# mhozza/covest

Hardware: AMD Instinct MI355X
Metric: grid-point log-likelihood evals/s, repeat model, 10k-bin hist (higher is better)
Workload: dtype f64

## Files before the change

### covest_amd/csrc/band.h

```cpp
#pragma once
#include <math.h>

#ifndef COVEST_HD
#ifdef __HIPCC__
#define COVEST_HD __host__ __device__
#else
#define COVEST_HD
#endif
#endif

namespace covest {

constexpr double kBandLn = 56.0;
constexpr int kBandClasses = 8;
constexpr int kBandNewton = 2;

constexpr int kBandMinShared = 8;

struct Band {
    int step_lo, step_hi;
};

struct BandTile {
    double key_first, key_last, cls_first, cls_last;
};

COVEST_HD inline BandTile band_tile(const double *ln_rate, const double *ln_comb, double key_first, double key_last)
{
    BandTile t = {key_first, key_last, -INFINITY, -INFINITY};
    for (int s = 1; s < kBandClasses; ++s) {
        const double lc = ln_comb[s] - ln_comb[0], lr = ln_rate[s] - ln_rate[0];
        if (!(lc > -INFINITY))
            continue;
        const double a = lc + key_first * lr, b = lc + key_last * lr;
// ... 14 lines not shown
    const Band full = {0, n_steps};
    const double mu = -ln_1mq, L = rate0 + mu;
    if (!(rate0 > 0.0) || !(mu >= 0.0) || !(L < 1e300) || !(t.key_first >= 1.0) || !(t.key_last >= t.key_first) ||
        !(t.key_last < 16384.0) || o_ref_max < 3 || n_steps < 2)
        return full;
    const double mode = t.key_last * mth.rcp(L);
    double o_ref = floor(mode);
    o_ref = o_ref < 3.0 ? 3.0 : o_ref;
    o_ref = o_ref > (double)o_ref_max ? (double)o_ref_max : o_ref;
    const double inv_ref = mth.rcp(o_ref);
    double a = 2.0 * mode + 8.0;
    for (int it = 0; it < kBandNewton; ++it) {
        const double g = -(a - o_ref) * L + t.key_last * mth.ln(a * inv_ref) + kBandLn;
        const double dg = -L + t.key_last * mth.rcp(a);
        if (!(dg < 0.0))
            return full;
        a -= g * mth.rcp(dg);
        if (!(a > mode))
            return full;
    }
    const double o_edge = ceil(a) + 1.0;
    if (!(o_edge < 4.0 * (double)n_steps))
        return full;
    const int step_hi = ((int)o_edge + 2) >> 2;
    if (step_hi < 1 || step_hi >= n_steps)
        return full;
    const double o_drop = 1.0 + 4.0 * (double)step_hi, o_top = 4.0 * (double)n_steps;
    const double base = o_ref * rate0 - (o_drop - o_ref) * mu + kBandLn, ln_o = mth.ln(o_top * inv_ref);
    if (!(base + t.key_first * ln_o + t.cls_first <= 0.0) || !(base + t.key_last * ln_o + t.cls_last <= 0.0))
        return full;
    return Band{0, step_hi};
}

struct BandBytes {
    static constexpr int kSlots = 6, kNone = 255;
    unsigned w0 = ~0u, w1 = ~0u;
    COVEST_HD void set(int k, int step_hi)
    {
        const unsigned hi = (unsigned)(step_hi < kNone ? step_hi : kNone);
        if (k < 4)
            w0 = (w0 & ~(255u << (8 * k))) | (hi << (8 * k));
        else
            w1 = (w1 & ~(255u << (8 * (k - 4)))) | (hi << (8 * (k - 4)));
    }
    COVEST_HD int get(int k) const { return (int)(((k < 4 ? w0 >> (8 * k) : w1 >> (8 * (k - 4)))) & 255u); }
};

}
```

### covest_amd/csrc/factored_build.h

```cpp
#pragma once
#include "factored_diag.h"
#include "fastmath.h"
#include "streams.h"
#include "tiles.h"
#include "wave.h"

namespace covest {

struct BuildLane {
    int tid, ld;
    bool in_row;
    __device__ __forceinline__ double *column(double *dst) const { return dst + (in_row ? tid : 0); }
};

template <int N, bool SPO, bool STORE>
__device__ __forceinline__ double walk_tile(StreamSet<8> &st, bool in_row, double *row, int ld, const double *scal, double k0,
                                            double renorm)
{
    if (STORE && !in_row)
        return 0.0;
    double xx[8];
#pragma unroll
    for (int s = 0; s < 8; ++s) {
        double xs = st.x[s];
// ... 79 lines not shown
        }
        return 0.0;
    }
    double sum = 0.0;
    for (int b = 0; b < (STORE ? kTileBins : nb); ++b) {
        const double g = b < nb ? st.step() : 0.0;
        if ((SPO || !STORE) && b < nb)
            sum = fma(g, scal[b], sum);
        if (STORE && ln.in_row)
            colp[b * ln.ld] = g;
    }
    st.leave_tile(rc.renorm);
    return SPO ? sum * 0x1p476 : sum * (1.0 / kBasicScale);
}

__device__ __forceinline__ bool sum_item_matters(const TileView &tv, const StreamSet<8> &st, int first, int n)
{
    const int tl = first + n - 1;
    const TileRec ra = tv.rec[first], rb = tv.rec[tl];
    const double ka = ra.k0 - 1.0, kb = rb.k0 + (double)(rb.nb - 1);
    const double lga = ra.lgam_prev, lgb = rb.lgam_last;
    bool matters = false;
#pragma unroll
    for (int s = 0; s < 8; ++s) {
        if ((st.gone >> s) & 1u)
            continue;
        const double lx = st.an.lx(s), c = st.an.c(s);
        const double top = fmax(fma(ka, lx, c - lga), fma(kb, lx, c - lgb));
        matters = matters || !(top < StreamSet<8>::kSumWindowLn) || (st.x[s] >= ka - 1.0 && st.x[s] <= kb + 1.0);
    }
    return __any(matters);
}

template <bool TAIL, bool SPO>
__device__ __forceinline__ void build_item(const TileView &tv, const FactoredPlan &plan, StreamSet<8> &st, CompSum &so,
                                           bool &resync, int tid, int ld, bool in_row, Stamps &stamps, int it,
                                           bool seg_start, double *dst)
{
    const BuildLane ln = {tid, ld, in_row};
    const int first = TAIL ? __builtin_amdgcn_readfirstlane(tv.item_first[it]) : it;
    if (TAIL && tv.item_sum[it] != 0) {
        if (COVEST_SKIP_PHASE(plan, 1))
            return;
        const int n = __builtin_amdgcn_readfirstlane(tv.item_ntiles[it]);
        if (SPO) {
            if (!seg_start && !sum_item_matters(tv, st, first, n)) {
#pragma unroll
                for (int s = 0; s < 8; ++s)
                    st.v[s] = 0.0;
                resync = true;
                return;
            }
            for (int r = 0; r < n; ++r) {
                if (st.gone == 0xFFu && !(seg_start && r == 0))
                    break;
                so.add(build_tile<SPO, false>(tv, plan, st, ln, stamps, first + r, (seg_start && r == 0) || resync, nullptr));
                resync = false;
            }
            return;
        }
        double *colp = ln.column(dst);
        for (int r = 0; r < n; ++r) {
            const double gsum = build_tile<SPO, false>(tv, plan, st, ln, stamps, first + r, seg_start && r == 0, nullptr);
            if (ln.in_row)
                colp[r * ln.ld] = gsum;
        }
        for (int r = n; r < kTileBins; ++r)
            if (ln.in_row)
                colp[r * ln.ld] = 0.0;
    } else {
        const double tsum = build_tile<SPO, true>(tv, plan, st, ln, stamps, first, seg_start || (SPO && resync), dst);
        resync = false;
        if (SPO)
            so.add(tsum);
    }
}

}
```

### covest_amd/csrc/factored_diag.h

```cpp
#pragma once
#include <hip/hip_runtime.h>

#include "tiles.h"

namespace covest {

struct StampNames {
    enum Lap {
        kBuild,
        kContract,
        kLog,
        kWait,
        kShared,
        kZero,
        kEnter,
        kFirst,
    };
    enum Stage {
        kStart,
        kFetched,
        kStreams,
        kUnits,
        kWalked,
    };
};

#ifdef COVEST_DIAG
struct Stamps : StampNames {
    long long *out;
    int mode;
    long long t0 = 0, lap_sum[8] = {0, 0, 0, 0, 0, 0, 0, 0}, at[5] = {0, 0, 0, 0, 0};
    __device__ Stamps(const FactoredPlan &plan, int waves, int wave)
        : out(plan.diag ? plan.diag + ((int64_t)(blockIdx.x * gridDim.y + blockIdx.y) * waves + wave) * 8 : nullptr),
          mode(plan.skip_phases)
    {
        stage(kStart);
    }
    __device__ void stage(Stage s) { at[s] = (long long)clock64(); }
    __device__ void walk_begins()
    {
        if (out)
            t0 = (long long)clock64();
    }
    __device__ void lap(Lap which)
    {
        if (out) {
            const long long now = (long long)clock64();
            lap_sum[which] += now - t0;
            t0 = now;
        }
    }
    __device__ void count_zero_tile()
    {
        if (out)
            lap_sum[kZero] += 1;
    }
    template <int MU>
    __device__ void first_fragments(const double (&a0)[MU], const double (&wfirst)[MU])
    {
        if (out) {
            double sink = 0.0;
#pragma unroll
            for (int k = 0; k < MU; ++k)
                sink += a0[k] + wfirst[k];
            asm volatile("" ::"v"(sink));
            lap(kFirst);
        }
    }
    __device__ void barrier_passed(int p, int t_begin, int t_end, int lane)
    {
        if (out && (mode & 0x10000)) {
            const long long now = (long long)clock64();
            if (lane == 0) {
                const int grp = (mode & 0x20000) ? min(7, p - t_begin + 1)
                                                 : min(7, (p - t_begin + 1) * 8 / (t_end - t_begin + 1));
                out[grp] += now - t0;
            }
        }
        lap(kWait);
    }
    __device__ void dump_laps(int lane)
    {
        stage(kWalked);
        if (out && lane == 0 && !(mode & 0x50000))
            for (int i = 0; i < 8; ++i)
                out[i] = lap_sum[i];
    }
    __device__ void dump_stages(int lane)
    {
        if (out && (mode & 0x40000) && lane == 0) {
            const long long end = (long long)clock64();
            for (int s = 0; s < 4; ++s)
                out[s] = at[s + 1] - at[s];
            out[4] = end - at[kWalked];
            out[5] = end - at[kStart];
            out[6] = at[kStart];
            out[7] = end;
        }
    }
};
#else
struct Stamps : StampNames {
    __device__ Stamps(const FactoredPlan &, int, int) {}
    __device__ void stage(Stage) {}
    __device__ void walk_begins() {}
    __device__ void lap(Lap) {}
    __device__ void count_zero_tile() {}
    template <int MU>
    __device__ void first_fragments(const double (&)[MU], const double (&)[MU])
    {
    }
    __device__ void barrier_passed(int, int, int, int) {}
    __device__ void dump_laps(int) {}
    __device__ void dump_stages(int) {}
};
#endif

}
```

### covest_amd/csrc/host_common.cpp

```cpp
#include "factored_launch.h"
#include "host.h"

using namespace covest;

namespace {
thread_local std::string g_last_error;
}

namespace covest {

int set_error(int code, const std::string &msg)
{
    g_last_error = msg;
    return code;
}

int fail_hip(hipError_t e, const char *what)
{
    g_last_error = std::string(what) + ": " + hipGetErrorString(e);
    if (e == hipErrorOutOfMemory) {
        (void)hipGetLastError();
        return COVEST_E_NOMEM;
    }
    return (e == hipErrorNoDevice || e == hipErrorInvalidDevice || e == hipErrorInsufficientDriver)
// ... 285 lines not shown
LaunchRecordScope::LaunchRecordScope(LaunchRecord &r) : prev(tls_record)
{
    r.clear();
    tls_record = &r;
}
LaunchRecordScope::LaunchRecordScope(LaunchRecord &r, bool append) : prev(tls_record)
{
    if (!append)
        r.clear();
    tls_record = &r;
}
LaunchRecordScope::~LaunchRecordScope() { tls_record = prev; }

void record_launch(const char *name, int64_t launches)
{
    LaunchRecord *r = tls_record;
    if (!r || launches <= 0)
        return;
    for (int i = 0; i < r->n_entries; ++i)
        if (r->entries[i].name == name) {
            r->entries[i].launches += launches;
            return;
        }
    if (r->n_entries < (int)(sizeof r->entries / sizeof r->entries[0]))
        r->entries[r->n_entries++] = LaunchRecord::Entry{name, launches};
}

void record_factored_plan(const FactoredPlan &plan, int shared_tiles, bool long_part)
{
    LaunchRecord *r = tls_record;
    if (!r || r->n_plans >= (int)(sizeof r->plans / sizeof r->plans[0]))
        return;
    r->plans[r->n_plans++] = LaunchRecord::Plan{plan.n_threads, plan.n_buf,  plan.ld,        plan.n_qblocks,
                                                shared_tiles,   plan.n_pass, plan.list_mode, long_part};
}

int64_t launch_record_text(const LaunchRecord &r, char *buf, int64_t cap)
{
    std::string t;
    char line[256];
    for (int i = 0; i < r.n_entries; ++i) {
        std::snprintf(line, sizeof line, "launch %s %lld\n", r.entries[i].name, (long long)r.entries[i].launches);
        t += line;
    }
    for (int i = 0; i < r.n_plans; ++i) {
        const LaunchRecord::Plan &p = r.plans[i];
        std::snprintf(line, sizeof line,
                      "plan n_threads=%d n_buf=%d ld=%d n_qblocks=%d shared_tiles=%d long=%d n_pass=%d list_mode=%d\n",
                      p.n_threads, p.n_buf, p.ld, p.n_qblocks, p.shared_tiles, p.long_part ? 1 : 0, p.n_pass, p.list_mode);
        t += line;
    }
    if (buf && cap > 0) {
        const size_t n = std::min<size_t>(t.size(), (size_t)(cap - 1));
        std::memcpy(buf, t.data(), n);
        buf[n] = '\0';
    }
    return (int64_t)t.size();
}

}

extern "C" {

int64_t covest_compiled_variants(char *buf, int64_t cap)
{
    if (cap < 0 || (cap > 0 && !buf))
        return fail(COVEST_E_INVALID, "covest_compiled_variants: bad argument");
    std::string t;
    auto add = [&](const char *const *names, int n) {
        for (int i = 0; i < n; ++i) {
            t += names[i];
            t += '\n';
        }
    };
    for (const FactoredVariant &v : kFactoredVariantTable)
        add(&v.name, 1);
    add(kFactoredFinishNames, 2);
    add(kBasicVariantNames, kBasicVariants);
    add(kFixVariantNames, kFixVariants);
    add(kArgminVariantNames, kArgminVariants);
    add(kDerivVariantNames, kDerivVariants);
    if (buf && cap > 0) {
// ... 33 lines not shown
```

### covest_amd/csrc/kernels.h

```cpp
#pragma once
#include <hip/hip_runtime_api.h>

#include <cstddef>

#include "device_model.h"
#include "handback.h"
#include "kmer_plan.h"
#include "tiles.h"

namespace covest {

struct LaunchRecord {
    struct Entry {
        const char *name;
        int64_t launches;
    };
    struct Plan {
        int32_t n_threads, n_buf, ld, n_qblocks, shared_tiles, n_pass, list_mode;
        bool long_part;
    };
    Entry entries[16];
    int n_entries = 0;
    Plan plans[8];
    int n_plans = 0;
    void clear() { n_entries = n_plans = 0; }
};
void record_launch(const char *name, int64_t launches = 1);
void record_factored_plan(const FactoredPlan &plan, int shared_tiles, bool long_part);
struct LaunchRecordScope {
    explicit LaunchRecordScope(LaunchRecord &r);
    LaunchRecordScope(LaunchRecord &r, bool append);
    ~LaunchRecordScope();
    LaunchRecord *prev;
};
constexpr int kFactoredVariants = 10, kBasicVariants = 8, kFixVariants = 6, kArgminVariants = 3, kDerivVariants = 7;
extern const char *const kFactoredFinishNames[2];
extern const char *const kBasicVariantNames[kBasicVariants];
extern const char *const kFixVariantNames[kFixVariants];
extern const char *const kArgminVariantNames[kArgminVariants];
extern const char *const kDerivVariantNames[kDerivVariants];

hipError_t launch_ll_direct(const DevModel &m, const PointSource &src, int64_t n, double *out_ll,
                            double *out_p, hipStream_t stream, bool ref_overflow = false);

hipError_t launch_ll_basic(const DevModel &m, const TileView &tv, const PointSource &src, int64_t n,
                           double *out_ll, const SubList &sub_list, hipStream_t stream);

hipError_t launch_ll_factored(const DevModel &m, const TileView &tv, const FactoredPlan &plan,
                              double *out_ll, const SubList &sub_list, hipStream_t stream);

hipError_t launch_ll_finish_partials(const DevModel &m, const TileView &tv, const double *partial,
                                     const int32_t *first_item, const double *point_par, const int32_t *point_T,
// ... 207 lines not shown
```

### covest_amd/csrc/ll_factored.hip

```cpp
#include <hip/hip_runtime.h>

#include <algorithm>
#include <mutex>

#include "band.h"
#include "factored_build.h"
#include "factored_contract.h"
#include "factored_diag.h"
#include "factored_epilogue.h"
#include "factored_launch.h"
#include "factored_log.h"
#include "fastmath.h"
#include "handback.h"
#include "kernels.h"
#include "point_fetch.h"
#include "streams.h"
#include "wave.h"

namespace covest {

namespace {

template <int NT, int HU, bool TAIL, bool PLAIN, int LDC = 0>
__global__ __launch_bounds__(NT) void ll_factored_kernel(const DevModel m, const int32_t n_tiles, const int32_t n_items,
                                                         const double *__restrict__ tile_dbl,
                                                         const int32_t *__restrict__ tile_int,
                                                         const FactoredPlan plan,
                                                         double *__restrict__ out_ll, const SubList sub_list)
{
    const TileView tv = tile_view_from(n_tiles, n_items, tile_dbl, tile_int);
    constexpr int NW = NT / kWave;
    constexpr int MU = 2 * HU;
    static_assert(MU == 6, "contract loops are written for 6 slots");
    constexpr bool SPO = PLAIN && TAIL;
    constexpr bool NEED_SCAL = !PLAIN;
    constexpr int LOG_DEG = PLAIN ? 3 : 5;
    const int LD = LDC ? LDC : plan.ld;
    constexpr int NE = FactoredLds::entries_of(NT);
    const FactoredLds lay{NT, plan.n_buf, LD, SPO};
    extern __shared__ double Gs[];
    __shared__ __attribute__((aligned(16))) double log_tab[kLogTableDoubles];
    __shared__ unsigned sub_rec[NE * 2];
    __shared__ __attribute__((aligned(16))) double2 rowc[2][kTileBins];
    __shared__ __attribute__((aligned(16))) double rows[NEED_SCAL ? 2 : 1][NEED_SCAL ? kTileBins : 2];
    __shared__ __attribute__((aligned(16))) double rho_tab[PLAIN ? NW * MU * 4 : 4];
    __shared__ double lconst_s;
    __shared__ double band_ln[PLAIN ? kBandClasses : 1];
    static_assert(MU == kMaxUnits, "the LDS layout counts kMaxUnits slots a wave");
    static_assert(sizeof(log_tab) + sizeof(sub_rec) + sizeof(rowc) + sizeof(rows) + sizeof(rho_tab) + sizeof(lconst_s) +
                          sizeof(band_ln) + 7 * 15 <= kFactoredStaticLds, "the planners' LDS budget (tiles.h) must hold the kernel's static LDS");

    const int tid = threadIdx.x;
    const int lane = tid & (kWave - 1);
    const int wave = __builtin_amdgcn_readfirstlane(tid / kWave);
    Stamps stamps(plan, NW, wave);
    const double p_clamp = plan.p_clamp;
    const double zero_frac = kZeroSteps * (kGridStep / p_clamp);
    const int list_mode = PLAIN ? 0 : plan.list_mode;

    const int n_seg = list_mode ? plan.n_seg : 1;
    const int unit = list_mode ? (int)blockIdx.x / n_seg : (int)blockIdx.x;
    const int seg = list_mode ? (int)blockIdx.x - unit * n_seg : 0;
    const int seg_items = (n_items + n_seg - 1) / n_seg;
    const int t_begin = seg * seg_items, t_end = min(n_items, t_begin + seg_items);
    const int64_t ce = (PLAIN || list_mode == 0) ? plan.ce_end - 1 - unit : plan.ce_begin + unit;
    const bool list = list_mode == 1 || list_mode == 2;
    const int64_t ic = list ? ce : ce / plan.n_e;
    const int64_t ie = list ? ce : ce - ic * plan.n_e;
    double par[kMaxParams] = {plan.c_axis[ic], plan.e_axis[ie], 0, 0, 0};
    constexpr int kLogPerThread = (kLogTableDoubles + NT - 1) / NT;
    double log_v[kLogPerThread];
#pragma unroll
    for (int u = 0; u < kLogPerThread; ++u)
        log_v[u] = kLogTable[min(tid + u * NT, kLogTableDoubles - 1)];
    const double rho_v = PLAIN ? plan.unit_rho[(int64_t)blockIdx.y * NW * MU * 4 + min(tid, NW * MU * 4 - 1)] : 0.0;
    double lc_first = 0.0;
    if (wave == NW - 1 && t_begin + lane < t_end)
        lc_first = tv.item_lconst[t_begin + lane];
#pragma unroll
    for (int u = 0; u < kLogPerThread; ++u)
        if (tid + u * NT < kLogTableDoubles)
            log_tab[tid + u * NT] = log_v[u];
    if (PLAIN && tid < NW * MU * 4)
// ... 1 lines not shown
#pragma unroll
    for (int u = 0; u < (NE + NT - 1) / NT; ++u)
        if (tid + u * NT < NE) {
            sub_rec[2 * (tid + u * NT)] = 0xFFFFFFFFu;
            sub_rec[2 * (tid + u * NT) + 1] = 0;
        }
    clamp_point<2>(m, par);
    const bool finite = isfinite(par[0]) && isfinite(par[1]);
    const int n_pass = PLAIN ? 1 : plan.n_pass;
    if (tid < 8 * n_pass)
        Gs[lay.rates() + tid] = error_class_rate_mul(m, par[0], par[1], tid, m.n_err);
    if (wave == NW - 1) {
        double lc = 0.0 + lc_first;
        for (int t = t_begin + lane + kWave; t < t_end; t += kWave)
            lc += tv.item_lconst[t];
        lc = wave_sum(lc);
        if (lane == 0)
            lconst_s = PLAIN ? lc - kLogRawBias<kScaleBits> * tv.suf_h[0] : lc;
    }
    __syncthreads();
    stamps.stage(Stamps::kFetched);

    const int my_pass = n_pass == 1 ? 0 : tid / plan.pass_stride;
    const int o_local = n_pass == 1 ? tid : tid - my_pass * plan.pass_stride;
    const bool wave_builds = wave * kWave < plan.n_columns;
    const int o_base = PLAIN ? 0 : list_mode == 2 ? plan.item_obase[ce] : plan.o_base;
    const int o_mine = o_base + o_local + 1;
    double lam[8];
#pragma unroll
    for (int s = 0; s < 8; ++s)
        lam[s] = Gs[lay.rates() + 8 * my_pass + s];
    if (PLAIN && tid < kBandClasses)
        band_ln[tid] = fast_log(Gs[lay.rates() + tid], log_tab);
    double n_total = -1.0;
    if (n_pass > 1) {
        n_total = 0.0;
        for (int s = 0; s < 8 * n_pass; ++s)
            n_total += m.comb[s] * (1.0 - exp_neg_rn((double)o_mine * Gs[lay.rates() + s]));
    }
    __syncthreads();
    StreamSet<8> st;
    if (wave_builds) {
        st.template init<false>(m, lam, o_mine, finite && my_pass < n_pass && o_local < plan.max_o, log_tab,
                                log_tab, 8 * my_pass, n_total);
    } else {
        st.gone = 0u;
#pragma unroll
        for (int s = 0; s < 8; ++s) {
            st.v[s] = 0.0;
            st.x[s] = 0.0;
            st.an.set(s, 0.0, -INFINITY);
        }
    }
    stamps.stage(Stamps::kStreams);
    const bool lane_in_row = tid < LD - 2;
    if (tid < FactoredLds::kSlack)
        Gs[lay.slack() + tid] = 0.0;
    if (tid < lay.rows()) {
        Gs[lay.pad(tid)] = 0.0;
        Gs[lay.pad(tid) + 1] = 0.0;
    }

    const int col = lane & 15;
    const int kq = lane >> 4;
    int len[MU], cont[MU], uhalf[MU], qslot[MU], cut[MU], a_off0[MU], nsh[MU];
    double r4[MU], llacc[MU];
// ... 29 lines not shown
        u_T[k] = plan.q_T[slot];
        r4[k] = plan.q_r4[slot];
    }
#pragma unroll
    for (int k = 0; k < MU; ++k) {
        const bool on = qslot[k] >= 0;
        const int first_step = __builtin_amdgcn_readfirstlane(u_s0[k]);
        len[k] = __builtin_amdgcn_readfirstlane(u_len[k]);
        cont[k] = __builtin_amdgcn_readfirstlane(u_cont[k]);
        uhalf[k] = __builtin_amdgcn_readfirstlane(u_half[k]);
        nsh[k] = PLAIN ? __builtin_amdgcn_readfirstlane(u_nsh[k]) : 0;
        a_off0[k] = (16 * uhalf[k] + col) * LD + kq + 4 * first_step;
        const int t_lane = on ? u_T[k] : 0;
        const int o0 = __builtin_amdgcn_readfirstlane(u_o0[k]);
        cut[k] = ((t_lane - (o0 + kq) + 3) >> 2) - nsh[k];
        llacc[k] = 0.0;
        dead[k] = 0;
        spacc[(TAIL && !SPO) ? k : 0].hi = 0.0;
        spacc[(TAIL && !SPO) ? k : 0].lo = 0.0;
    }

    unsigned m_first = 0, m_cont = 0, m_sh = 0;
#pragma unroll
    for (int k = 0; k < MU; ++k) {
        m_first |= (qslot[k] >= 0 && !cont[k]) ? 1u << k : 0u;
        m_cont |= cont[k] ? 1u << k : 0u;
        m_sh |= nsh[k] > 0 ? 1u << k : 0u;
    }
    BandBytes bands;
    bool wave_bands = false;
#pragma unroll
    for (int k = 0; k < MU; ++k)
        wave_bands = wave_bands || (PLAIN && !wave_builds && nsh[k] >= kBandMinShared);
    if (PLAIN && wave_bands) {
        struct {
            const double *tab;
            __device__ double ln(double x) const { return fast_log(x, tab); }
            __device__ double rcp(double x) const
            {
                const double r = __builtin_amdgcn_rcp(x);
                return fma(fma(-x, r, 1.0), r, r);
            }
        } const mth = {log_tab};
        const int it = min(lane, t_end - 1);
        const double key_first = tv.rec[TAIL ? tv.item_first[it] : it].k0;
        const double key_last = (lane < kWave - 1 ? key_first : tv.rec[n_tiles - 1].k0) + (double)(kTileBins - 1);
        const BandTile bt = band_tile(band_ln, m.ln_comb, key_first, key_last);
#pragma unroll
        for (int k = 0; k < MU; ++k) {
            if (nsh[k] < kBandMinShared)
                continue;
            const Band b = band_of_unit(mth, lam[0], rho_tab[4 * (wave * MU + k) + 1], 4 + 4 * nsh[k], nsh[k] + len[k], bt);
            bands.set(k, b.step_hi);
        }
    }
    double wfirst[MU], wrun[MU];
    auto load_weights = [&]() {
#pragma unroll
        for (int k = 0; k < MU; ++k) {
            const double2 pw = reinterpret_cast<const double2 *>(plan.piece_w)[(int64_t)(slot_base + k) * kWave + lane];
            wfirst[k] = pw.x;
            wrun[k] = pw.y;
        }
    };
    load_weights();

    bool resync = false;
    auto build = [&](int it, bool seg_start, double *dst) __attribute__((always_inline)) {
        build_item<TAIL, SPO>(tv, plan, st, so, resync, tid, LD, lane_in_row, stamps, it, seg_start, dst);
    };
    stamps.walk_begins();
    stamps.stage(Stamps::kUnits);

    const bool dbuf = plan.n_buf == 2;
    double nxt_h = 0.0, nxt_c = 0.0, nxt_s = 0.0;
    auto fetch_rows = [&](int it) {
        if (tid < kTileBins && it < t_end) {
            const int64_t at = (int64_t)it * kTileBins + tid;
            nxt_h = tv.item_cnt[at];
            nxt_c = tv.item_iscal[at];
            if (NEED_SCAL)
                nxt_s = tv.item_scal[at];
        }
    };
    int last_item = t_end - 1;
    if (SPO)
        while (last_item > t_begin && tv.item_sum[last_item] != 0)
            --last_item;
    const bool last_first = PLAIN && t_end - t_begin >= 2 && last_item > t_begin;
    auto tile_at = [&](int p) -> int { return last_first ? (p == t_begin ? last_item : (p <= last_item ? p - 1 : p)) : p; };
    const int t_endx = t_end + (SPO ? 1 : 0);
    fetch_rows(tile_at(t_begin));
    for (int p = t_begin - (dbuf ? 1 : 0); p < t_endx; ++p) {
        const int pb = dbuf ? p + 1 : p;
        if (SPO && pb == t_end) {
            if (wave_builds && lane_in_row) {
                double *dst = Gs + lay.buf(pb) + tid;
                dst[0] = so.hi * 0x1p-540;
                dst[LD] = so.lo * 0x1p-540;
            }
        } else if (pb < t_end) {
            if (tid < kTileBins) {
                rowc[pb & 1][tid] = make_double2(nxt_h, p_clamp * nxt_c);
                if (NEED_SCAL)
                    rows[pb & 1][tid] = nxt_s;
            }
            fetch_rows(pb + 1 < t_end ? tile_at(pb + 1) : t_end);
            if (wave_builds) {
                if (last_first && pb == t_begin + 1)
                    st.gone = 0u;
                build(tile_at(pb), pb == t_begin || (last_first && (pb == t_begin + 1 || pb == last_item + 1)), Gs + lay.buf(pb));
            }
        }
        stamps.lap(Stamps::kBuild);
        if (!dbuf)
            __syncthreads();
        const bool sp_item = SPO && p == t_end;
        if (p >= t_begin && !(SPO && !sp_item && tv.item_sum[tile_at(p)] != 0)) {
            const int t = tile_at(p);
            const double *cur = Gs + lay.buf(p);
            d4 acc[MU];
            const d4 zero4 = (d4){0.0, 0.0, 0.0, 0.0};
            double a0[MU];
#pragma unroll
            for (int k = 0; k < MU; ++k)
                a0[k] = cur[a_off0[k]];
            BandBytes item_bands;
            if (PLAIN && !sp_item)
                item_bands = bands_of_item(bands, t);
            stamps.first_fragments(a0, wfirst);
#pragma unroll
            for (int k = 0; k < MU; ++k) {
                if (!PLAIN || !((m_sh >> k) & 1u) || COVEST_SKIP_PHASE(plan, 8)) {
                    acc[k] = len[k] > 0 ? __builtin_amdgcn_mfma_f64_16x16x4f64(a0[k], wfirst[k], zero4, 0, 0, 0) : zero4;
                    continue;
                }
                const double rr16 = rho_tab[4 * (wave * MU + k)];
                const double2 rt = *reinterpret_cast<const double2 *>(&rho_tab[4 * (wave * MU + k) + 2]);
                const double rr4 = rt.x, rho_n = rt.y;
                const double *g1 = cur + a_off0[k];
                int nsh_k = nsh[k];
                asm volatile("" : "+s"(nsh_k));
                if (PLAIN)
                    nsh_k = min(nsh_k, item_bands.get(k) - 1);
// ... 303 lines not shown
```

### covest_amd/csrc/plan_factored.cpp

```cpp
#include "host.h"

#include <initializer_list>

using namespace covest;

namespace covest {

double copy_number_weight_host(double q1, double q2, double q, int o)
{
    if (o == 1)
        return q1;
    if (o == 2)
        return (1 - q1) * q2;
    return (1 - q1) * (1 - q2) * q * std::pow(1 - q, (double)(o - 3));
}

namespace {

constexpr int kQTileSlots = 16;
constexpr int kStepColumns = 4;
constexpr int kStepLanes = kStepColumns * kQTileSlots;
static_assert(kStepLanes == 64, "one wave holds the weights of a step");
static_assert(2 * kHalfUnits == kMaxUnits, "a wave's slots are two halves' (tiles.h)");
constexpr int mfma_steps_of(int columns) { return (columns + kStepColumns - 1) / kStepColumns; }

struct UnitTables {
    std::vector<int32_t> tile, half, s0, o0, len, cont, nsh, pair;
    explicit UnitTables(size_t n) : tile(n, -1), half(n, 0), s0(n, 0), o0(n, 1), len(n, 0), cont(n, 0), nsh(n, 0), pair(n, -1) {}
    size_t size() const { return tile.size(); }
    void set(size_t at, int tile_, int half_, int s0_, int o0_, int len_, bool cont_, int nsh_)
    {
        tile[at] = tile_;
        half[at] = half_;
        s0[at] = s0_;
        o0[at] = o0_;
        len[at] = len_;
        cont[at] = cont_ ? 1 : 0;
        nsh[at] = nsh_;
    }
};

class PlanPack {
  public:
    enum Array { Axes, QR4, PieceW, UnitRho, QT, QOrig, UnitTile, UnitHalf, UnitS0, UnitO0, UnitLen, UnitCont, UnitNsh, UnitPair, kArrays };
    PlanPack(std::initializer_list<std::pair<Array, const std::vector<double> *>> dbl,
             std::initializer_list<std::pair<Array, const std::vector<int32_t> *>> ints)
    {
        for (const auto &d : dbl)
            add(d.first, d.second->data(), d.second->size() * sizeof(double));
        for (const auto &i : ints)
            add(i.first, i.second->data(), i.second->size() * sizeof(int32_t));
    }
    size_t bytes() const { return bytes_; }
    void stage(char *dst) const
    {
        for (int k = 0; k < n_; ++k) {
            const Part &p = part_[order_[k]];
            if (p.bytes)
                std::memcpy(dst + p.off, p.src, p.bytes);
        }
    }
    void bind(const void *device_base) { base_ = static_cast<const char *>(device_base); }
    const double *f64(Array a) const { return static_cast<const double *>(at(a)); }
    const int32_t *i32(Array a) const { return static_cast<const int32_t *>(at(a)); }

  private:
    struct Part {
        const void *src = nullptr;
        size_t off = 0, bytes = 0;
        bool listed = false;
    };
    void add(Array a, const void *src, size_t bytes)
    {
        part_[a] = Part{src, bytes_, bytes, true};
        order_[n_++] = a;
        bytes_ += bytes;
    }
// ... 33 lines not shown
    return COVEST_OK;
}

struct PartGeometry {
    int max_o;
    int pass_stride;
    int n_columns, ld, n_buf;
    int n_threads, units_per_wave, n_qblocks;
    int n_waves() const { return n_threads / 64; }
    size_t block_slots() const { return (size_t)n_waves() * kMaxUnits; }
    size_t n_unit() const { return (size_t)n_qblocks * block_slots(); }
};

void fill_plan(FactoredPlan &pl, const PartGeometry &geo, int n_pass, const PlanPack &pack)
{
    pl = FactoredPlan{};
    pl.max_o = geo.max_o;
    pl.n_pass = n_pass;
    pl.pass_stride = geo.pass_stride;
    pl.n_columns = geo.n_columns;
    pl.n_threads = geo.n_threads;
    pl.half_units = kHalfUnits;
    pl.n_qblocks = geo.n_qblocks;
    pl.ld = geo.ld;
    pl.n_buf = geo.n_buf;
    pl.unit_tile = pack.i32(PlanPack::UnitTile);
    pl.unit_half = pack.i32(PlanPack::UnitHalf);
    pl.unit_s0 = pack.i32(PlanPack::UnitS0);
    pl.unit_o0 = pack.i32(PlanPack::UnitO0);
    pl.unit_len = pack.i32(PlanPack::UnitLen);
    pl.unit_cont = pack.i32(PlanPack::UnitCont);
    pl.unit_nsh = pack.i32(PlanPack::UnitNsh);
    pl.unit_pair = pack.i32(PlanPack::UnitPair);
    pl.unit_rho = pack.f64(PlanPack::UnitRho);
    pl.piece_w = pack.f64(PlanPack::PieceW);
    pl.q_r4 = pack.f64(PlanPack::QR4);
    pl.q_T = pack.i32(PlanPack::QT);
    pl.q_orig = pack.i32(PlanPack::QOrig);
    pl.n_seg = 1;
}

struct QOrder {
    int64_t n1, n2, n3, nq;
    std::vector<int32_t> order;
    std::vector<int32_t> tile_nsh;
    int32_t n_qtiles;
    int t_max;
};

struct PartSpec {
    int32_t tile_lo, tile_hi;
    int o_base, chunk, n_pass, list_mode;
    int32_t n_qtiles() const { return tile_hi - tile_lo; }
};

struct SlotQ {
    double q1, q2, q;
};

struct PartColumns {
    std::vector<int32_t> q_t, q_orig;
    std::vector<double> r4;
    std::vector<SlotQ> w;
    std::vector<int32_t> nsteps, nsh;
    int t_loc_max = 1;
    int mfma_steps(int qt) const { return (int)nsteps[(size_t)qt] - (int)nsh[(size_t)qt]; }
// ... 204 lines not shown
            if (d < kStepColumns && o0 + d >= (int)pc.q_t[ls])
                w = 0.0;
            if (d < kStepColumns || nsh == 0)
                piece_w[(at * kStepLanes + (size_t)((d % kStepColumns) * kQTileSlots + colx)) * 2 + (size_t)(d / kStepColumns)] = w;
        }
        if (nsh > 0) {
            unit_rho[4 * at] = pw_16;
            unit_rho[4 * at + 1] = std::log(base);
            unit_rho[4 * at + 2] = pw_4;
            unit_rho[4 * at + 3] = pw_inv;
            double g2 = pw_after;
            for (int d = 0; d < kStepColumns; ++d, g2 *= base)
                piece_w[(at * kStepLanes + (size_t)(d * kQTileSlots + colx)) * 2 + 1] = head * g2;
        }
    }
}

void pair_halves(UnitTables &ut, size_t block_slots)
{
    for (size_t b0 = 0; b0 < ut.size(); b0 += block_slots) {
        const size_t b1 = b0 + block_slots;
        for (size_t at = b0; at < b1; ++at) {
            if (ut.tile[at] < 0 || ut.half[at] != 0 || ut.cont[at])
                continue;
            for (size_t at2 = b0; at2 < b1; ++at2)
                if (ut.tile[at2] == ut.tile[at] && ut.half[at2] == 1 && !ut.cont[at2]) {
                    ut.pair[at] = (int32_t)(at2 - b0);
                    break;
                }
        }
    }
}

void apply_diag_env(FactoredPlan &pl)
{
#ifdef COVEST_DIAG
    if (std::getenv("COVEST_FACTORED_NBUF"))
        pl.n_buf = std::max(1, std::min(pl.n_buf, std::atoi(std::getenv("COVEST_FACTORED_NBUF"))));
    const char *skip = std::getenv("COVEST_FACTORED_SKIP");
    pl.skip_phases = skip ? std::atoi(skip) : 0;
    if (pl.list_mode == 0 && std::getenv("COVEST_FACTORED_DIAG")) {
        void *dp = nullptr;
        const size_t bytes = (size_t)(pl.ce_end - pl.ce_begin) * pl.n_qblocks * (pl.n_threads / 64) * 8 * sizeof(long long);
        if (hipMalloc(&dp, bytes) == hipSuccess && hipMemset(dp, 0, bytes) == hipSuccess) {
            pl.diag = static_cast<long long *>(dp);
            if (std::atoi(std::getenv("COVEST_FACTORED_DIAG")) >= 2)
                pl.skip_phases |= 0x10000;
            if (std::atoi(std::getenv("COVEST_FACTORED_DIAG")) == 3)
                pl.skip_phases |= 0x20000;
            if (std::atoi(std::getenv("COVEST_FACTORED_DIAG")) == 4)
                pl.skip_phases = (pl.skip_phases & ~0x10000) | 0x40000;
            std::fprintf(stderr, "COVEST_FACTORED_DIAG %p %zu\n", dp, bytes);
        }
    }
#else
    (void)pl;
#endif
}

int build_plan_part(covest_grid *g, const double *const *axes, const std::vector<int32_t> &t_table, const QOrder &qo,
                    const PartSpec &ps, const Charges &ch, DevBuf &buf, FactoredPlan &pl, std::vector<int32_t> *q_orig_out)
{
    const covest_model *m = g->model;
    const PartColumns pc = part_columns(m, axes, t_table, qo, ps);
    if (q_orig_out)
        *q_orig_out = pc.q_orig;
    const PartGeometry geo =
        part_geometry(pc.t_loc_max, ps.n_pass, ps.n_qtiles(), std::max<int64_t>(1, g->len[0] * g->len[1]));
    UnitTables ut(geo.n_unit());
    for (int blk = 0; blk < geo.n_qblocks; ++blk) {
        const int rc = deal_qblock(blk, ps, pc, geo, ch, ut);
        if (rc != COVEST_OK)
            return rc;
    }
    std::vector<double> piece_w(ut.size() * kStepLanes * 2, 0.0), unit_rho(ut.size() * 4, 1.0);
    for (size_t at = 0; at < ut.size(); ++at)
        if (ut.tile[at] >= 0)
            slot_weights(at, ps, pc, ut, piece_w.data(), unit_rho.data());
    pair_halves(ut, geo.block_slots());
    PlanPack pack({{PlanPack::QR4, &pc.r4}, {PlanPack::PieceW, &piece_w}, {PlanPack::UnitRho, &unit_rho}},
                  {{PlanPack::QT, &pc.q_t}, {PlanPack::QOrig, &pc.q_orig}, {PlanPack::UnitTile, &ut.tile},
                   {PlanPack::UnitHalf, &ut.half}, {PlanPack::UnitS0, &ut.s0}, {PlanPack::UnitO0, &ut.o0},
                   {PlanPack::UnitLen, &ut.len}, {PlanPack::UnitCont, &ut.cont}, {PlanPack::UnitNsh, &ut.nsh},
                   {PlanPack::UnitPair, &ut.pair}});
    const int rc = upload_to_grid(g, buf, pack);
    if (rc != COVEST_OK)
        return rc;
    fill_plan(pl, geo, ps.n_pass, pack);
    pl.c_axis = g->src.axis[0];
    pl.e_axis = g->src.axis[1];
    pl.n_e = g->len[1];
    pl.n_q = qo.nq;
    pl.ce_begin = g->flat_begin / qo.nq;
    pl.ce_end = (g->flat_end + qo.nq - 1) / qo.nq;
    pl.n_qtiles = ps.n_qtiles();
    pl.o_base = ps.o_base;
    pl.flat_begin = g->flat_begin;
    pl.flat_end = g->flat_end;
    pl.list_mode = ps.list_mode;
    pl.p_clamp = clamp_for(m, qo.t_max);
    pl.ce_first = pl.ce_begin;
    pl.n_cols_partial = (int64_t)ps.n_qtiles() * kQTileSlots;
    apply_diag_env(pl);
    return COVEST_OK;
}

struct ByThreshold {
    const std::vector<int32_t> &t_table;
    bool operator()(int32_t a, int32_t b) const { return t_table[(size_t)a] > t_table[(size_t)b]; }
};

bool wants_shared_order(const QOrder &qo, int n_pass)
{
    const int64_t group = qo.n1 * qo.n2, group_padded = (group + kQTileSlots - 1) / kQTileSlots * kQTileSlots;
    bool share = n_pass == 1 && 3 * (group_padded - group) <= group;
#ifdef COVEST_DIAG
    if (const char *share_env = std::getenv("COVEST_FACTORED_SHARE"))
        share = share && std::atoi(share_env) != 0;
#endif
    return share;
}

QOrder plain_order(QOrder qo, const std::vector<int32_t> &t_table)
{
    std::vector<int32_t> all((size_t)qo.nq);
    for (int64_t i = 0; i < qo.nq; ++i)
        all[(size_t)i] = (int32_t)i;
    std::stable_sort(all.begin(), all.end(), ByThreshold{t_table});
    qo.n_qtiles = (int32_t)((qo.nq + kQTileSlots - 1) / kQTileSlots);
    qo.order.assign((size_t)qo.n_qtiles * kQTileSlots, -1);
    std::copy(all.begin(), all.end(), qo.order.begin());
    qo.tile_nsh.assign((size_t)qo.n_qtiles, 0);
    return qo;
}

// ... 243 lines not shown
```

### covest_amd/csrc/tiles.h

```cpp
#pragma once
#include <hip/hip_runtime_api.h>
#include <stdint.h>

namespace covest {

constexpr int kTileBins = 32;
constexpr int kScaleBits = 540;
constexpr double kScaleLn = 540.0 * 0.693147180559945309417232121458;
constexpr double kWindowLn = -760.0;
constexpr int kBasicShift = 64;
constexpr double kBasicScale = 0x1p64;

struct alignas(64) TileRec {
    double k0, lgam_prev, lgam_last, renorm;
    int32_t nb, run_start, all_zero, has_filler;
    double pad[2];
};
static_assert(sizeof(TileRec) == 64, "one cache line");

struct TileView {
    int32_t n_tiles;
    int32_t n_items;
    const double *dbl_base;
    const int32_t *int_base;
// ... 51 lines not shown
    tv.item_lconst = tv.item_iscal + (int64_t)ni * kTileBins;
    tv.suf_h = tv.item_lconst + ni;
    tv.suf_jh = tv.suf_h + (nt + 1);
    tv.suf_lgh = tv.suf_jh + (nt + 1);
    tv.suf_first = tv.suf_lgh + (nt + 1);
    tv.suf_first_lg = tv.suf_first + (nt + 1);
    tv.last_key = tv.suf_first_lg + (nt + 1);
    tv.n_bins = ints;
    tv.run_start = ints + nt;
    tv.all_zero = ints + 2 * (int64_t)nt;
    tv.has_filler = ints + 3 * (int64_t)nt;
    tv.item_first = ints + 4 * (int64_t)nt;
    tv.item_ntiles = tv.item_first + ni;
    tv.item_sum = tv.item_ntiles + ni;
    tv.row_bin = tv.item_sum + ni;
    tv.rec = reinterpret_cast<const TileRec *>(dbl + tile_arrays_dbl(nt, ni));
    return tv;
}

constexpr int kMaxUnits = 6;
constexpr int kHalfUnits = 3;
constexpr int kBuildCost = 27;
constexpr int kBuildCostLowKeys = 24;
constexpr int kLowKeyTile = 384;
#ifndef COVEST_LIST_SEGMENTS
#define COVEST_LIST_SEGMENTS 16
#endif
constexpr int kListSegments = COVEST_LIST_SEGMENTS;
constexpr int kMinPieceSteps = 6;
constexpr int kSharedStepsPerMfma = 4;
constexpr int kMinSharedSteps = 3;
constexpr int kLastBuilderExtra = 4;
constexpr int kUnitOverhead = 2;

struct FactoredPlan {
    const double *c_axis, *e_axis;
    int64_t n_e;
    int64_t ce_begin, ce_end;
    int64_t n_q;
    int32_t n_qtiles;
    int32_t max_o;
    int32_t n_pass;
    int32_t pass_stride;
    int32_t n_columns;
    int32_t o_base;
    int32_t n_threads;
    int32_t half_units;
    int32_t n_qblocks;
    int32_t ld;
    int32_t n_buf;
    const int32_t *unit_tile;
    const int32_t *unit_half;
    const int32_t *unit_s0;
    const int32_t *unit_o0;
    const int32_t *unit_len;
    const int32_t *unit_cont;
    const int32_t *unit_nsh;
    const int32_t *unit_pair;
    const double *unit_rho;
    const double *piece_w;
    const int32_t *qtile_nsteps;
    const int32_t *qtile_nfull;
    const int32_t *q_T;
    const int32_t *q_orig;
    const double *q_first8;
    const double *q_r4;
    int64_t flat_begin, flat_end;
    int32_t list_mode;
    double p_clamp;
    int32_t n_seg;
    const int32_t *item_obase;
    double *partial;
    int64_t ce_first;
    int64_t n_cols_partial;
    long long *diag;
    int32_t skip_phases;
};

constexpr int kLdsBytes = 160 * 1024;
constexpr int kFactoredStaticLds = 13440;

constexpr __host__ __device__ int factored_ld(int columns) { return (columns + kTileBins - 1) / kTileBins * kTileBins + 2; }

struct FactoredLds {
    int nt, n_buf, ld;
    bool spo;
    static constexpr int kSlack = 64;
    static constexpr int kRates = 32;
    __host__ __device__ static constexpr int entries_of(int nt) { return nt / 64 * kMaxUnits * 16; }
    __host__ __device__ constexpr int entries() const { return entries_of(nt); }
    __host__ __device__ constexpr int rows() const { return n_buf * kTileBins; }
    __host__ __device__ constexpr int buf(int b) const { return n_buf == 2 ? (b & 1) * kTileBins * ld : 0; }
    __host__ __device__ constexpr int pad(int row) const { return row * ld + ld - 2; }
    __host__ __device__ constexpr int slack() const { return n_buf * kTileBins * ld; }
    __host__ __device__ constexpr int rates() const { return 0; }
    __host__ __device__ constexpr bool spo_inside() const
    {
        return kTileBins * ld >= (n_buf == 2 ? 0 : 2 * ld) + 3 * entries();
    }
    __host__ __device__ constexpr int spo_parts(int t_end) const
    {
        return !spo_inside() ? slack() + kSlack : n_buf == 2 ? buf(t_end + 1) + entries() : 2 * ld + entries();
    }
    __host__ __device__ constexpr int part_ll() const { return 0; }
    __host__ __device__ constexpr int part_hi(int t_end) const { return spo ? spo_parts(t_end) : entries(); }
    __host__ __device__ constexpr int part_lo(int t_end) const { return part_hi(t_end) + entries(); }
    __host__ __device__ constexpr int total() const
// ... 17 lines not shown
```

Before: 438.8 million.

## Skip building tile columns above band-limited column ceiling per block

Computes a per-block column ceiling from the band limits of the units that consume each tile (plus a host-computed floor and a few extra band units evaluated by non-building waves). Builder waves whose columns all lie above the ceiling skip the tile walk, zero their buffer once and force a stream resync. The aim is to avoid building Poisson-like columns that the banded consumers never read. In exchange it adds an LDS atomicMax pass, extra band evaluations, host planning and more plan state, and correctness depends on the ceiling being conservative.

New measurement: 465.6 million (median of 6 runs). 1.06x the previous value.

```diff
diff --git a/covest_amd/csrc/band.h b/covest_amd/csrc/band.h
--- a/covest_amd/csrc/band.h
+++ b/covest_amd/csrc/band.h
@@ -1,5 +1,6 @@
 #pragma once
 #include <math.h>
+#include <stdint.h>
 
 #ifndef COVEST_HD
 #ifdef __HIPCC__
@@ -80,6 +81,44 @@
     return Band{0, step_hi};
 }
 
+COVEST_HD inline int band_top_column(const Band &b) { return 4 * b.step_hi; }
+
+inline int column_limit_of_block(const int32_t *tile, const int32_t *nsh, const int32_t *cont, const int32_t *top, int n_waves,
+                                 int slots_per_wave, int n_build, bool plain, int floor_min, int32_t *extra, int n_extra_max)
+{
+    const bool bands = plain && n_build < n_waves;
+    int floor = floor_min, n_made = 0, n_extra = 0;
+    int32_t made[64];
+    for (int j = 0; j < n_extra_max; ++j)
+        extra[j] = -1;
+    for (int round = 0; round < 2; ++round)
+        for (int w = round == 0 ? n_build : 0; w < (round == 0 ? n_waves : (n_build < n_waves ? n_build : n_waves)); ++w)
+            for (int k = 0; k < slots_per_wave; ++k) {
+                const int at = w * slots_per_wave + k;
+                if (tile[at] < 0)
+                    continue;
+                bool has_band = false;
+                if (bands && nsh[at] >= kBandMinShared && !cont[at] && !(k + 1 < slots_per_wave && tile[at + 1] == tile[at] && cont[at + 1])) {
+                    bool known = false;
+                    for (int i = 0; i < n_made; ++i)
+                        known = known || made[i] == tile[at];
+                    if (round == 0 || known) {
+                        has_band = true;
+                    } else if (n_extra < n_extra_max) {
+                        extra[n_extra++] = at;
+                        has_band = true;
+                    }
+                    if (has_band && !known && n_made < 64)
+                        made[n_made++] = tile[at];
+                    else if (has_band && !known)
+                        has_band = round == 0;
+                }
+                if (!has_band)
+                    floor = floor > top[tile[at]] ? floor : top[tile[at]];
+            }
+    return floor;
+}
+
 struct BandBytes {
     static constexpr int kSlots = 6, kNone = 255;
     unsigned w0 = ~0u, w1 = ~0u;
diff --git a/covest_amd/csrc/factored_build.h b/covest_amd/csrc/factored_build.h
--- a/covest_amd/csrc/factored_build.h
+++ b/covest_amd/csrc/factored_build.h
@@ -135,10 +135,10 @@
     return __any(matters);
 }
 
-template <bool TAIL, bool SPO>
+template <bool TAIL, bool SPO, bool SKIP>
 __device__ __forceinline__ void build_item(const TileView &tv, const FactoredPlan &plan, StreamSet<8> &st, CompSum &so,
-                                           bool &resync, int tid, int ld, bool in_row, Stamps &stamps, int it,
-                                           bool seg_start, double *dst)
+                                           bool &resync, unsigned &zeroed, int tid, int ld, bool in_row, Stamps &stamps, int it,
+                                           bool seg_start, bool skip, int buf_bit, double *dst)
 {
     const BuildLane ln = {tid, ld, in_row};
     const int first = TAIL ? __builtin_amdgcn_readfirstlane(tv.item_first[it]) : it;
@@ -172,7 +172,26 @@
             if (ln.in_row)
                 colp[r * ln.ld] = 0.0;
     } else {
-        const double tsum = build_tile<SPO, true>(tv, plan, st, ln, stamps, first, seg_start || (SPO && resync), dst);
+        if (SKIP && skip) {
+            if (!((zeroed >> buf_bit) & 1u)) {
+                zeroed |= 1u << buf_bit;
+                if (ln.in_row) {
+                    double *colp = ln.column(dst);
+#pragma unroll
+                    for (int b = 0; b < kTileBins; ++b)
+                        colp[b * ln.ld] = 0.0;
+                }
+            }
+#pragma unroll
+            for (int s = 0; s < 8; ++s)
+                st.v[s] = 0.0;
+            resync = true;
+            stamps.count_skipped_item();
+            return;
+        }
+        if (SKIP)
+            zeroed &= ~(1u << buf_bit);
+        const double tsum = build_tile<SPO, true>(tv, plan, st, ln, stamps, first, seg_start || ((SPO || SKIP) && resync), dst);
         resync = false;
         if (SPO)
             so.add(tsum);
diff --git a/covest_amd/csrc/factored_diag.h b/covest_amd/csrc/factored_diag.h
--- a/covest_amd/csrc/factored_diag.h
+++ b/covest_amd/csrc/factored_diag.h
@@ -55,6 +55,11 @@
         if (out)
             lap_sum[kZero] += 1;
     }
+    __device__ void count_skipped_item()
+    {
+        if (out)
+            lap_sum[kZero] += 1ll << 20;
+    }
     template <int MU>
     __device__ void first_fragments(const double (&a0)[MU], const double (&wfirst)[MU])
     {
@@ -106,6 +111,7 @@
     __device__ void walk_begins() {}
     __device__ void lap(Lap) {}
     __device__ void count_zero_tile() {}
+    __device__ void count_skipped_item() {}
     template <int MU>
     __device__ void first_fragments(const double (&)[MU], const double (&)[MU])
     {
diff --git a/covest_amd/csrc/host_common.cpp b/covest_amd/csrc/host_common.cpp
--- a/covest_amd/csrc/host_common.cpp
+++ b/covest_amd/csrc/host_common.cpp
@@ -341,7 +341,8 @@
     if (!r || r->n_plans >= (int)(sizeof r->plans / sizeof r->plans[0]))
         return;
     r->plans[r->n_plans++] = LaunchRecord::Plan{plan.n_threads, plan.n_buf,  plan.ld,        plan.n_qblocks,
-                                                shared_tiles,   plan.n_pass, plan.list_mode, long_part};
+                                                shared_tiles,   plan.n_pass, plan.list_mode, long_part,
+                                                plan.col_floor};
 }
 
 int64_t launch_record_text(const LaunchRecord &r, char *buf, int64_t cap)
@@ -355,8 +356,8 @@
     for (int i = 0; i < r.n_plans; ++i) {
         const LaunchRecord::Plan &p = r.plans[i];
         std::snprintf(line, sizeof line,
-                      "plan n_threads=%d n_buf=%d ld=%d n_qblocks=%d shared_tiles=%d long=%d n_pass=%d list_mode=%d\n",
-                      p.n_threads, p.n_buf, p.ld, p.n_qblocks, p.shared_tiles, p.long_part ? 1 : 0, p.n_pass, p.list_mode);
+                      "plan n_threads=%d n_buf=%d ld=%d n_qblocks=%d shared_tiles=%d long=%d n_pass=%d list_mode=%d col_floor=%d\n",
+                      p.n_threads, p.n_buf, p.ld, p.n_qblocks, p.shared_tiles, p.long_part ? 1 : 0, p.n_pass, p.list_mode, p.col_floor);
         t += line;
     }
     if (buf && cap > 0) {
diff --git a/covest_amd/csrc/kernels.h b/covest_amd/csrc/kernels.h
--- a/covest_amd/csrc/kernels.h
+++ b/covest_amd/csrc/kernels.h
@@ -18,6 +18,7 @@
     struct Plan {
         int32_t n_threads, n_buf, ld, n_qblocks, shared_tiles, n_pass, list_mode;
         bool long_part;
+        int32_t col_floor;
     };
     Entry entries[16];
     int n_entries = 0;
diff --git a/covest_amd/csrc/ll_factored.hip b/covest_amd/csrc/ll_factored.hip
--- a/covest_amd/csrc/ll_factored.hip
+++ b/covest_amd/csrc/ll_factored.hip
@@ -46,9 +46,10 @@
     __shared__ __attribute__((aligned(16))) double rho_tab[PLAIN ? NW * MU * 4 : 4];
     __shared__ double lconst_s;
     __shared__ double band_ln[PLAIN ? kBandClasses : 1];
+    __shared__ int col_hi[PLAIN ? kWave : 1];
     static_assert(MU == kMaxUnits, "the LDS layout counts kMaxUnits slots a wave");
     static_assert(sizeof(log_tab) + sizeof(sub_rec) + sizeof(rowc) + sizeof(rows) + sizeof(rho_tab) + sizeof(lconst_s) +
-                          sizeof(band_ln) + 7 * 15 <= kFactoredStaticLds, "the planners' LDS budget (tiles.h) must hold the kernel's static LDS");
+                          sizeof(band_ln) + sizeof(col_hi) + 8 * 15 <= kFactoredStaticLds, "the planners' LDS budget (tiles.h) must hold the kernel's static LDS");
 
     const int tid = threadIdx.x;
     const int lane = tid & (kWave - 1);
@@ -116,6 +117,8 @@
         lam[s] = Gs[lay.rates() + 8 * my_pass + s];
     if (PLAIN && tid < kBandClasses)
         band_ln[tid] = fast_log(Gs[lay.rates() + tid], log_tab);
+    if (PLAIN && tid >= NT - kWave)
+        col_hi[tid - (NT - kWave)] = plan.col_floor;
     double n_total = -1.0;
     if (n_pass > 1) {
         n_total = 0.0;
@@ -211,7 +214,8 @@
 #pragma unroll
     for (int k = 0; k < MU; ++k)
         wave_bands = wave_bands || (PLAIN && !wave_builds && nsh[k] >= kBandMinShared);
-    if (PLAIN && wave_bands) {
+    const bool wave_limit = PLAIN && !wave_builds && plan.col_floor < plan.max_o;
+    if (PLAIN && (wave_bands || wave_limit)) {
         struct {
             const double *tab;
             __device__ double ln(double x) const { return fast_log(x, tab); }
@@ -225,12 +229,30 @@
         const double key_first = tv.rec[TAIL ? tv.item_first[it] : it].k0;
         const double key_last = (lane < kWave - 1 ? key_first : tv.rec[n_tiles - 1].k0) + (double)(kTileBins - 1);
         const BandTile bt = band_tile(band_ln, m.ln_comb, key_first, key_last);
+        int hi = 0;
 #pragma unroll
         for (int k = 0; k < MU; ++k) {
             if (nsh[k] < kBandMinShared)
                 continue;
             const Band b = band_of_unit(mth, lam[0], rho_tab[4 * (wave * MU + k) + 1], 4 + 4 * nsh[k], nsh[k] + len[k], bt);
             bands.set(k, b.step_hi);
+            hi = max(hi, band_top_column(b));
+        }
+        if (wave_limit) {
+            const int n_build_waves = (plan.n_columns + kWave - 1) / kWave;
+#pragma unroll 1
+            for (int j = wave - n_build_waves; j < kBandExtra; j += NW - n_build_waves) {
+                const int e = __builtin_amdgcn_readfirstlane(plan.band_extra[(int)blockIdx.y * kBandExtra + j]);
+                if (e < 0)
+                    continue;
+                const int at = (int)blockIdx.y * NW * MU + e;
+                const int nsh_x = __builtin_amdgcn_readfirstlane(plan.unit_nsh[at]);
+                const int len_x = __builtin_amdgcn_readfirstlane(plan.unit_len[at]);
+                const Band b = band_of_unit(mth, lam[0], rho_tab[4 * e + 1], 4 + 4 * nsh_x, nsh_x + len_x, bt);
+                hi = max(hi, band_top_column(b));
+            }
+            if (hi > 0)
+                atomicMax(&col_hi[lane], hi);
         }
     }
     double wfirst[MU], wrun[MU];
@@ -245,8 +267,9 @@
     load_weights();
 
     bool resync = false;
-    auto build = [&](int it, bool seg_start, double *dst) __attribute__((always_inline)) {
-        build_item<TAIL, SPO>(tv, plan, st, so, resync, tid, LD, lane_in_row, stamps, it, seg_start, dst);
+    unsigned zeroed = 0;
+    auto build = [&](int it, bool seg_start, bool skip, int buf_bit, double *dst) __attribute__((always_inline)) {
+        build_item<TAIL, SPO, PLAIN>(tv, plan, st, so, resync, zeroed, tid, LD, lane_in_row, stamps, it, seg_start, skip, buf_bit, dst);
     };
     stamps.walk_begins();
     stamps.stage(Stamps::kUnits);
@@ -288,7 +311,12 @@
             if (wave_builds) {
                 if (last_first && pb == t_begin + 1)
                     st.gone = 0u;
-                build(tile_at(pb), pb == t_begin || (last_first && (pb == t_begin + 1 || pb == last_item + 1)), Gs + lay.buf(pb));
+                const int it = tile_at(pb);
+                bool skip = false;
+                if (PLAIN && pb > t_begin)
+                    skip = wave * kWave + 1 > __builtin_amdgcn_readfirstlane(col_hi[min(it, kWave - 1)]);
+                build(it, pb == t_begin || (last_first && (pb == t_begin + 1 || pb == last_item + 1)), skip, dbuf ? pb & 1 : 0,
+                      Gs + lay.buf(pb));
             }
         }
         stamps.lap(Stamps::kBuild);
diff --git a/covest_amd/csrc/plan_factored.cpp b/covest_amd/csrc/plan_factored.cpp
--- a/covest_amd/csrc/plan_factored.cpp
+++ b/covest_amd/csrc/plan_factored.cpp
@@ -1,3 +1,4 @@
+#include "band.h"
 #include "host.h"
 
 #include <initializer_list>
@@ -42,7 +43,7 @@
 
 class PlanPack {
   public:
-    enum Array { Axes, QR4, PieceW, UnitRho, QT, QOrig, UnitTile, UnitHalf, UnitS0, UnitO0, UnitLen, UnitCont, UnitNsh, UnitPair, kArrays };
+    enum Array { Axes, QR4, PieceW, UnitRho, QT, QOrig, UnitTile, UnitHalf, UnitS0, UnitO0, UnitLen, UnitCont, UnitNsh, UnitPair, BandExtra, kArrays };
     PlanPack(std::initializer_list<std::pair<Array, const std::vector<double> *>> dbl,
              std::initializer_list<std::pair<Array, const std::vector<int32_t> *>> ints)
     {
@@ -142,6 +143,8 @@
     pl.unit_cont = pack.i32(PlanPack::UnitCont);
     pl.unit_nsh = pack.i32(PlanPack::UnitNsh);
     pl.unit_pair = pack.i32(PlanPack::UnitPair);
+    pl.band_extra = pack.i32(PlanPack::BandExtra);
+    pl.col_floor = geo.max_o;
     pl.unit_rho = pack.f64(PlanPack::UnitRho);
     pl.piece_w = pack.f64(PlanPack::PieceW);
     pl.q_r4 = pack.f64(PlanPack::QR4);
@@ -412,6 +415,23 @@
     }
 }
 
+int column_limit(const PartSpec &ps, const PartColumns &pc, const PartGeometry &geo, const UnitTables &ut, std::vector<int32_t> &extra)
+{
+    std::vector<int32_t> top((size_t)ps.n_qtiles(), 0);
+    for (size_t ls = 0; ls < pc.q_t.size(); ++ls)
+        top[ls / kQTileSlots] = std::max(top[ls / kQTileSlots], pc.q_t[ls] - 1);
+    const bool plain = ps.list_mode == 0 && ps.n_pass == 1;
+    const int n_build = std::min(geo.n_waves(), (geo.n_columns + 63) / 64);
+    extra.assign((size_t)geo.n_qblocks * kBandExtra, -1);
+    int floor = 1;
+    for (int blk = 0; blk < geo.n_qblocks; ++blk) {
+        const size_t b0 = (size_t)blk * geo.block_slots();
+        floor = std::max(floor, column_limit_of_block(&ut.tile[b0], &ut.nsh[b0], &ut.cont[b0], top.data(), geo.n_waves(), kMaxUnits,
+                                                      n_build, plain, 1, &extra[(size_t)blk * kBandExtra], kBandExtra));
+    }
+    return floor;
+}
+
 void apply_diag_env(FactoredPlan &pl)
 {
 #ifdef COVEST_DIAG
@@ -458,11 +478,13 @@
         if (ut.tile[at] >= 0)
             slot_weights(at, ps, pc, ut, piece_w.data(), unit_rho.data());
     pair_halves(ut, geo.block_slots());
+    std::vector<int32_t> band_extra;
+    const int col_floor = column_limit(ps, pc, geo, ut, band_extra);
     PlanPack pack({{PlanPack::QR4, &pc.r4}, {PlanPack::PieceW, &piece_w}, {PlanPack::UnitRho, &unit_rho}},
                   {{PlanPack::QT, &pc.q_t}, {PlanPack::QOrig, &pc.q_orig}, {PlanPack::UnitTile, &ut.tile},
                    {PlanPack::UnitHalf, &ut.half}, {PlanPack::UnitS0, &ut.s0}, {PlanPack::UnitO0, &ut.o0},
                    {PlanPack::UnitLen, &ut.len}, {PlanPack::UnitCont, &ut.cont}, {PlanPack::UnitNsh, &ut.nsh},
-                   {PlanPack::UnitPair, &ut.pair}});
+                   {PlanPack::UnitPair, &ut.pair}, {PlanPack::BandExtra, &band_extra}});
     const int rc = upload_to_grid(g, buf, pack);
     if (rc != COVEST_OK)
         return rc;
@@ -481,6 +503,7 @@
     pl.p_clamp = clamp_for(m, qo.t_max);
     pl.ce_first = pl.ce_begin;
     pl.n_cols_partial = (int64_t)ps.n_qtiles() * kQTileSlots;
+    pl.col_floor = col_floor;
     apply_diag_env(pl);
     return COVEST_OK;
 }
diff --git a/covest_amd/csrc/tiles.h b/covest_amd/csrc/tiles.h
--- a/covest_amd/csrc/tiles.h
+++ b/covest_amd/csrc/tiles.h
@@ -107,6 +107,7 @@
 constexpr int kMinSharedSteps = 3;
 constexpr int kLastBuilderExtra = 4;
 constexpr int kUnitOverhead = 2;
+constexpr int kBandExtra = 4;
 
 struct FactoredPlan {
     const double *c_axis, *e_axis;
@@ -148,6 +149,8 @@
     double *partial;
     int64_t ce_first;
     int64_t n_cols_partial;
+    int32_t col_floor;
+    const int32_t *band_extra;
     long long *diag;
     int32_t skip_phases;
 };
```
